# Jasonlai0821/fftw3

Measured on AMD Instinct MI355X. Metric: GFLOPS (5N*log2N) + achieved HBM GB/s, 1D complex double N=2^20 batch=4096, higher is better.
Workload: dtype f64; 1 GPU; c2c n=1048576 howmany=4096 per GPU, forward, out-of-place, FFTW_ESTIMATE; parallelism=batch-sharded x1

## Files before the change

fftw3_amd/csrc/fa_hip.h:

```cpp
#ifndef FA_HIP_H
#define FA_HIP_H

#include <stddef.h>
#include "fftw3_amd.h"

#ifdef __cplusplus
extern "C" {
#endif

int   fa_hip_device_count(void);
int   fa_hip_rr_tile(int L);
int   fa_hip_r3t_tile(int L);
int   fa_hip_r3tw_rdec(int L);
int   fa_hip_r2c_rows_tile(int L);
int   fa_hip_r2c_rows1_tile(int L);
int   fa_hip_r2c_rows2m_tile(int L);
int   fa_hip_r2c_rows3_tile(int L);
int   fa_hip_r3_tile(int L);
int   fa_hip_blue_nb(int need);
int   fa_hip_blue_tile(int nb);
int   fa_hip_r1_tile(int L);
void *fa_hip_malloc(size_t nbytes);
void  fa_hip_free(void *p);
void *fa_hip_host_malloc(size_t nbytes);
int   fa_hip_host_free(void *p);
int   fa_hip_is_device_ptr(const void *p);
int   fa_hip_ptr_device(const void *p);
void  fa_hip_memcpy_h2d(void *dst, const void *src, size_t nbytes, void *stream);
void  fa_hip_memcpy_d2h(void *dst, const void *src, size_t nbytes, void *stream);
void  fa_hip_memset(void *dst, int v, size_t nbytes, void *stream);
void  fa_hip_stream_sync(void *stream);
void *fa_hip_event_create(void);
void  fa_hip_event_record(void *ev, void *stream);
float fa_hip_event_elapsed_ms(void *start, void *stop);
void  fa_hip_event_destroy(void *ev);
void *fa_hip_stream_create(void);
void  fa_hip_stream_destroy(void *stream);
void  fa_hip_stream_wait_event(void *stream, void *ev);
int   fa_hip_get_device(void);
void  fa_hip_set_device(int dev);
int   fa_hip_enable_peer(int dev, int peer);
void  fa_hip_memcpy_peer(void *dst, int dst_dev, const void *src, int src_dev, size_t nbytes, void *stream);
void  fa_hip_memcpy2d_peer(void *dst, size_t dpitch, const void *src, size_t spitch, size_t width, size_t height, void *stream);
size_t fa_hip_max_pitch(int dev);

int   fa_hip_slab_twiddle(double *p, long long rows, long long width, long long row_stride, long long c0,
                          long long n, int sign, const void *lo, const void *hi, int shift, void *stream);

int fa_hip_launch_step(const fftw_amd_step_desc *desc, double *const *bufs,
                       void *const *tables, long long chunk_start, long long chunk_n,
                       void *stream);

int fa_hip_launch_pair1024(const fftw_amd_step_desc *d_second, double *const *bufs_second,
                           long long cs2, long long cn2,
                           const fftw_amd_step_desc *d_first, double *const *bufs_first,
                           long long cs1, long long cn1, void *const *tables, void *stream);

// ... 5 lines not shown
```

fftw3_amd/csrc/fa_plan.h:

```cpp
#ifndef FA_PLAN_H
#define FA_PLAN_H

#include <stddef.h>
#include <pthread.h>
#include "fftw3.h"
#include "fftw3_amd.h"

typedef long long i64;

#define FA_MAXRANK 8
#define FA_MAXLOOPS 7
#define FA_MAXBUF 16
#define FA_MAXTAB 256
#define FA_MAXPASS 4
#define FA_MAXLANES 4

#define FA_PRIME_LDS_MAX 31

#define FA_TILE_ELEMS 4096
#define FA_LMAX_SINGLE 4096
#define FA_LDS_ELEMS 5120

enum { FA_C2C = 0, FA_R2C = 1, FA_C2R = 2, FA_R2R = 3 };
#define FA_REAL_IN(t)  ((t) == FA_R2C || (t) == FA_R2R)
#define FA_REAL_OUT(t) ((t) == FA_C2R || (t) == FA_R2R)

enum {
    FA_TAB_STAGE = 1,
    FA_TAB_TW_LO,
    FA_TAB_TW_HI,
    FA_TAB_CHIRP,
    FA_TAB_BLUE_SEQ,
    FA_TAB_RADER_SEQ,
    FA_TAB_DFT_OF,
    FA_TAB_PERM
};

typedef struct {
    int kind;
    i64 n;
    i64 aux;
    i64 len;
    int src;
    void *host;
    void *dev;
} fa_table;

typedef struct { i64 n, is, os; } fa_dim;

typedef struct {
    size_t chunk_bytes;
    int pipeline;
    int lmax_multi;
    int small_tiles;
    int long_first;
    int lanes;
    i64 tile_elems;
    int real_dec;
} fa_cfg;

typedef struct {
    int buf;
    i64 base;
    i64 im;
} fa_loc;

typedef struct {
    i64 n;
    i64 is, os;
    fa_loc src, dst;
    int nloops;
    fa_dim loops[FA_MAXLOOPS];
    int batch_loop;
    int flags_in, flags_out;
    int dense;
} fa_axis;

struct fftw_plan_s {
    int type;
    int kinds[FA_MAXRANK];
    fa_cfg cfg;
    int sign;
    unsigned flags;
    int rank;
    fa_dim dims[FA_MAXRANK];
    int hrank;
    fa_dim hdims[FA_MAXRANK];
    i64 in_im, out_im;

    fftw_amd_step_desc *steps;
    int nsteps, cap_steps;

    fa_table tabs[FA_MAXTAB];
    int ntabs;

    int nbufs;
    i64 buf_reals[FA_MAXBUF];
    int buf_busy[FA_MAXBUF];
    double *dbuf[FA_MAXBUF];

    i64 batch, chunk;

    double *ri, *ii, *ro, *io;
    i64 in_lo, in_hi, out_lo, out_hi;
    i64 out_written;
    int inplace;
    int single_chunk;
    int via_scratch;

    void *stream;
    int dev_ready;
    pthread_mutex_t lock;

    int nslots, split;
    int pair;
    int lanes;
    void *pstream[FA_MAXLANES];
    void *ev_a[4], *ev_b[4], *ev_begin, *ev_end[FA_MAXLANES];
    int failed;

    void *hstream[2];
    double *stage_in, *stage_out;
    size_t stage_in_bytes, stage_out_bytes;

    double est_flops;

    struct fftw_plan_s *alt;

    double *prof_ms;
    long long *prof_launches;
};

void fa_cexp(i64 m, i64 n, double out[2]);
i64  fa_mulmod(i64 x, i64 y, i64 p);
i64  fa_power_mod(i64 b, i64 e, i64 p);
int  fa_prime_factors(i64 n, i64 *primes, int *mult);
int  fa_is_prime(i64 n);
i64  fa_largest_prime_factor(i64 n);
i64  fa_find_generator(i64 p);
int  fa_lds_able(i64 n);
i64  fa_next_smooth(i64 n);
int  fa_radices(i64 L, int *rad);
int  fa_factor_passes(i64 n, int max_passes, i64 lmax_single, i64 lmax_multi, i64 *lens);
int  fa_factor_passes_pref(i64 n, int max_passes, i64 lmax_single, i64 lmax_multi, i64 *lens,
                           int (*tuned)(i64));

struct fftw_plan_s *fa_plan_new(void);
void fa_plan_free(struct fftw_plan_s *p);
int  fa_build(struct fftw_plan_s *p);
int  fa_device_init(struct fftw_plan_s *p);
void fa_run(struct fftw_plan_s *p, double *ri, double *ii, double *ro, double *io);
char *fa_sprint(const struct fftw_plan_s *p);
fa_cfg fa_default_cfg(void);

struct fftw_plan_s *fa_unaligned_twin(const struct fftw_plan_s *p);

#define FA_SLAB_MAXDEV 32
struct fa_slab1d;
void fa_slab1d_execute(struct fa_slab1d *d);
void fa_slab1d_sync(struct fa_slab1d *d);
void fa_slab1d_destroy(struct fa_slab1d *d);
fftw_plan fa_slab1d_local_plan(const struct fa_slab1d *d, int g, int which);
struct fftw_amd_slab_plan_s *fa_slab_wrap1d(struct fa_slab1d *d, int ndev);

#endif
```

fftw3_amd/csrc/hostmath.c:

```c
#include <math.h>
#include <stdlib.h>
#include <string.h>
#include "fa_plan.h"

void fa_cexp(i64 m, i64 n, double out[2]) {
    const double two_pi = 6.2831853071795864769252867665590057683943388;
    i64 full = 4 * n;
    i64 q = n;
    i64 a;
    int flip_s = 0, rot = 0, swap = 0;
    m %= n;
    if (m < 0) m += n;
    a = 4 * m;
    if (a > full - a) { a = full - a; flip_s = 1; }
    if (a > q) { a -= q; rot = 1; }
    if (a > q - a) { a = q - a; swap = 1; }
    {
        double th = (two_pi * (double)a) / (double)full;
        double c = cos(th), s = sin(th), t;
        if (swap) { t = c; c = s; s = t; }
        if (rot) { t = c; c = -s; s = t; }
        if (flip_s) s = -s;
        out[0] = c;
        out[1] = s;
    }
}

i64 fa_mulmod(i64 x, i64 y, i64 p) {
    return (i64)(((unsigned __int128)x * (unsigned __int128)y) % (unsigned __int128)p);
}

i64 fa_power_mod(i64 b, i64 e, i64 p) {
    i64 r = 1 % p;
    b %= p;
    if (b < 0) b += p;
    while (e > 0) {
        if (e & 1) r = fa_mulmod(r, b, p);
        b = fa_mulmod(b, b, p);
        e >>= 1;
    }
    return r;
}

int fa_prime_factors(i64 n, i64 *primes, int *mult) {
    int k = 0;
    i64 d;
    for (d = 2; d * d <= n; d += (d == 2 ? 1 : 2)) {
        if (n % d == 0) {
            primes[k] = d;
            mult[k] = 0;
            while (n % d == 0) { n /= d; ++mult[k]; }
            ++k;
        }
    }
    if (n > 1) { primes[k] = n; mult[k] = 1; ++k; }
    return k;
}

int fa_is_prime(i64 n) {
    i64 d;
    if (n < 2) return 0;
    for (d = 2; d * d <= n; d += (d == 2 ? 1 : 2))
        if (n % d == 0) return 0;
    return 1;
}

i64 fa_largest_prime_factor(i64 n) {
    i64 pr[64];
    int mu[64];
    int k = fa_prime_factors(n, pr, mu);
    return k ? pr[k - 1] : 1;
}

i64 fa_find_generator(i64 p) {
    i64 pr[64];
    int mu[64];
    int k, i;
    i64 g;
    if (p == 2) return 1;
    k = fa_prime_factors(p - 1, pr, mu);
// ... 174 lines not shown
```

fftw3_amd/csrc/kernels.hip:

```cpp
#include <string.h>
#include "common.hpp"

#include "pass1024.hpp"


struct PassArgs {
    const double *src;
    double *dst;
    i64 src_im, dst_im;
    i64 is_l, os_l;
    i64 dn[FFTW_AMD_MAX_DIMS], dis[FFTW_AMD_MAX_DIMS], dos[FFTW_AMD_MAX_DIMS], dtw[FFTW_AMD_MAX_DIMS];
    const cplx *wL;
    const cplx *tw_lo;
    const cplx *tw_hi;
    i64 tw_n;
    i64 ntiles;
    int tw_shift;
    int L, nrad;
    int rad[FFTW_AMD_MAX_RADICES];
    int ndims, T, ld, flags;
    int in_t_fast, out_t_fast;
    int lo_n;
    i64 lo_is, lo_os;
};
// ... 991 lines not shown
    if (e != hipSuccess) (void)hipGetLastError();
    FA_CHECK(hipSetDevice(cur));
    return (e == hipSuccess || e == hipErrorPeerAccessAlreadyEnabled) ? 0 : 1;
}
extern "C" void fa_hip_memcpy_peer(void *dst, int dst_dev, const void *src, int src_dev, size_t n, void *stream) {
    if (dst_dev == src_dev) FA_CHECK(hipMemcpyAsync(dst, src, n, hipMemcpyDeviceToDevice, (hipStream_t)stream));
    else FA_CHECK(hipMemcpyPeerAsync(dst, dst_dev, src, src_dev, n, (hipStream_t)stream));
}
extern "C" void fa_hip_memcpy2d_peer(void *dst, size_t dpitch, const void *src, size_t spitch, size_t width, size_t height, void *stream) {
    if (!width || !height) return;
    FA_CHECK(hipMemcpy2DAsync(dst, dpitch, src, spitch, width, height, hipMemcpyDeviceToDevice, (hipStream_t)stream));
}
extern "C" void fa_hip_stream_wait_event(void *s, void *ev) {
    FA_CHECK(hipStreamWaitEvent((hipStream_t)s, (hipEvent_t)ev, 0));
}


static void grid_for(i64 total, dim3 *grid) {
    i64 blocks = (total + 255) / 256;
    if (blocks < 1) blocks = 1;
    if (blocks > 256 * 32) blocks = 256 * 32;
    *grid = dim3((unsigned)blocks, 1, 1);
}


static std::atomic<unsigned> g_lds_attr_done{0};

template <bool VIN, bool VOUT>
static void launch_pass_variant(const PassArgs &pa, dim3 grid, size_t lds, hipStream_t st) {
    static int nth = 0;
    if (!nth) { const char *e = getenv("FFTW_AMD_GENERIC_THREADS"); nth = e ? atoi(e) : 256; if (nth < 64 || nth > 256) nth = 256; }
    hipLaunchKernelGGL((pass_generic_kernel<VIN, VOUT>), grid, dim3(nth), lds, st, pa);
}

int fa_launch_pass3tw(const fftw_amd_step_desc *d, double *const *bufs, void *const *tables,
                      i64 cs, i64 cn, hipStream_t st);
int fa_launch_pass3gw(const fftw_amd_step_desc *d, double *const *bufs, void *const *tables,
                      i64 cs, i64 cn, hipStream_t st);
int fa_launch_pass3g(const fftw_amd_step_desc *d, double *const *bufs, void *const *tables,
                     i64 cs, i64 cn, hipStream_t st);
int fa_launch_pass3t(const fftw_amd_step_desc *d, double *const *bufs, void *const *tables,
                     i64 cs, i64 cn, hipStream_t st);
int fa_launch_r2crows(const fftw_amd_step_desc *d, double *const *bufs, void *const *tables,
                      i64 cs, i64 cn, hipStream_t st);
int fa_launch_pass3s(const fftw_amd_step_desc *d, double *const *bufs, void *const *tables,
                     i64 cs, i64 cn, hipStream_t st);
int fa_launch_passrr(const fftw_amd_step_desc *d, double *const *bufs, void *const *tables,
                     i64 cs, i64 cn, hipStream_t st);
int fa_launch_blue(const fftw_amd_step_desc *d, double *const *bufs, void *const *tables,
                   i64 cs, i64 cn, hipStream_t st);
int fa_launch_pass1r(const fftw_amd_step_desc *d, double *const *bufs, void *const *tables,
                     i64 cs, i64 cn, hipStream_t st);

template <bool IN_T, bool OUT_T, int HAS_TW>
static void launch_p1024_variant(const P1024Args &pa, dim3 grid, hipStream_t st) {
    static std::atomic<unsigned> attr_done{0};
    const size_t lds = FA_P1024_LDS_DOUBLES * sizeof(double);
    if (fa_attr_needed(attr_done)) {
        FA_CHECK(hipFuncSetAttribute((const void *)pass1024_kernel<IN_T, OUT_T, HAS_TW>,
                                     hipFuncAttributeMaxDynamicSharedMemorySize, (int)lds));
        fa_attr_set(attr_done);
    }
    hipLaunchKernelGGL((pass1024_kernel<IN_T, OUT_T, HAS_TW>), grid, dim3(256), lds, st, pa);
}

static int fill_p1024(const fftw_amd_step_desc *d, double *const *bufs, void *const *tables,
                      i64 cs, i64 cn, P1024Args &pa, i64 *nblocks_out, bool *in_t, bool *out_t, int *tw) {
    int bd = d->batch_dim;
    i64 sbase = d->src_base, dbase = d->dst_base;
    if (d->L != 1024 || d->src_im != 1 || d->dst_im != 1 ||
        (d->flags & (FFTW_AMD_F_REAL_IN | FFTW_AMD_F_REAL_OUT | FFTW_AMD_F_CONJ_OUT)))
        return 1;
    for (int i = 0; i < FFTW_AMD_MAX_DIMS; ++i) {
        pa.dn[i] = (i < d->ndims) ? d->dim_n[i] : 1;
        pa.dis[i] = (i < d->ndims) ? d->dim_is[i] : 0;
        pa.dos[i] = (i < d->ndims) ? d->dim_os[i] : 0;
        pa.dtw[i] = (i < d->ndims) ? d->dim_tw[i] : 0;
    }
    if (bd >= 0) {
        sbase += chunk_adv(d->src_buf, cs, d->dim_is[bd]);
        dbase += chunk_adv(d->dst_buf, cs, d->dim_os[bd]);
        pa.dn[bd] = cn;
    }
    pa.src = bufs[d->src_buf] + sbase;
    pa.dst = bufs[d->dst_buf] + dbase;
    pa.is_l = d->is_l;
    pa.os_l = d->os_l;
    if (((uintptr_t)pa.src % 16) || ((uintptr_t)pa.dst % 16) || (pa.is_l % 2) || (pa.os_l % 2)) return 1;
    for (int i = 0; i < d->ndims; ++i)
        if ((pa.dis[i] % 2) || (pa.dos[i] % 2)) return 1;
    pa.w1024 = (const cplx *)tables[d->table];
    pa.tw_shift = d->tw_shift;
    pa.tw_lo = d->tw_n ? (const cplx *)tables[d->tw_lo] : NULL;
    pa.tw_hi = d->tw_n ? (const cplx *)tables[d->tw_hi] : NULL;
    pa.ndims = d->ndims;
    pa.flags = d->flags;
    pa.lo_sh = 0; pa.lo_is = d->tile_lo_is; pa.lo_os = d->tile_lo_os;
    pa.dbg = NULL;
    if (d->tile_lo_n > 1) {
        if (d->tile_lo_n != 2 && d->tile_lo_n != 4) return 1;
        pa.lo_sh = d->tile_lo_n == 2 ? 1 : 2;
        if ((pa.lo_is % 2) || (pa.lo_os % 2)) return 1;
    }
    pa.ntiles = (pa.dn[0] + (8 >> pa.lo_sh) - 1) / (8 >> pa.lo_sh);
    i64 nblocks = pa.ntiles;
    for (int i = 1; i < d->ndims; ++i) nblocks *= pa.dn[i];
    if (nblocks > 0x7fffffffLL) return 1;
    *nblocks_out = nblocks < 0 ? 0 : nblocks;
    *in_t = pa.dn[0] > 1 && iabs64(pa.dis[0]) <= iabs64(pa.is_l);
    *out_t = pa.dn[0] > 1 && iabs64(pa.dos[0]) <= iabs64(pa.os_l);
    *tw = d->tw_n == 0 ? 0 : ((d->flags & FFTW_AMD_F_TW_IN) ? 2 : 1);
    return 0;
}

static int launch_p1024(const fftw_amd_step_desc *d, double *const *bufs, void *const *tables,
                        i64 cs, i64 cn, hipStream_t st) {
    P1024Args pa;
    i64 nblocks = 0;
    bool in_t, out_t;
    int tw;
    if (fill_p1024(d, bufs, tables, cs, cn, pa, &nblocks, &in_t, &out_t, &tw)) return 1;
    if (nblocks <= 0) return 0;
    dim3 grid((unsigned)nblocks, 1, 1);
#define FA_P1024_CASE(I, O, W) if (in_t == I && out_t == O && tw == W) { launch_p1024_variant<I, O, W>(pa, grid, st); return 0; }
    FA_P1024_CASE(true, true, 0)  FA_P1024_CASE(true, true, 1)  FA_P1024_CASE(true, true, 2)
    FA_P1024_CASE(false, true, 0) FA_P1024_CASE(false, true, 1) FA_P1024_CASE(false, true, 2)
    FA_P1024_CASE(true, false, 0) FA_P1024_CASE(true, false, 1) FA_P1024_CASE(true, false, 2)
    FA_P1024_CASE(false, false, 0) FA_P1024_CASE(false, false, 1) FA_P1024_CASE(false, false, 2)
#undef FA_P1024_CASE
    return 1;
}

template <bool IN_T, bool OUT_T, int HAS_TW>
FA_DEV void p1024_block(const P1024Args &a, unsigned b0, unsigned nb, double *plane) {
    unsigned blk = (nb & 7) ? b0 : (b0 & 7) * (nb >> 3) + (b0 >> 3);
    const unsigned nt = (unsigned)a.ntiles;
    unsigned rest = blk / nt;
    const unsigned tile = blk - rest * nt;
    i64 soff = 0, doff = 0, twb = 0;
    for (int d = 1; d < a.ndims; ++d) {
        const unsigned dn = (unsigned)a.dn[d];
        const unsigned q = rest / dn, idx = rest - q * dn;
        rest = q;
        soff += (i64)idx * a.dis[d];
        doff += (i64)idx * a.dos[d];
        twb += (i64)idx * a.dtw[d];
    }
    const i64 t0 = (i64)tile * 8;
    P1024Tile t;
    t.lo_sh = 0; t.lo_is = 0; t.lo_os = 0;
    t.src = a.src + soff + t0 * a.dis[0];
    t.dst = a.dst + doff + t0 * a.dos[0];
    t.is_l = a.is_l; t.os_l = a.os_l;
    t.dis0 = a.dis[0]; t.dos0 = a.dos[0];
    t.dtw0 = a.dtw[0]; t.q0 = twb + t0 * a.dtw[0];
    t.w1024 = a.w1024; t.tw_lo = a.tw_lo; t.tw_hi = a.tw_hi; t.tw_shift = a.tw_shift;
    t.Tcur = (int)((a.dn[0] - t0 < 8) ? (a.dn[0] - t0) : 8);
    t.flags = a.flags;
    t.dbg = NULL;
    p1024_tile<IN_T, OUT_T, HAS_TW, 0>(t, plane, threadIdx.x);
}

__global__ void __launch_bounds__(256, 2)
pass1024_pair_kernel(const P1024Args a2, const P1024Args a1, const unsigned n2, const unsigned n1) {
    extern __shared__ __attribute__((aligned(16))) double plane[];
    if (blockIdx.x < n2) p1024_block<false, true, 2>(a2, blockIdx.x, n2, plane);
    else p1024_block<true, true, 0>(a1, blockIdx.x - n2, n1, plane);
}

extern "C" int fa_hip_launch_pair1024(const fftw_amd_step_desc *d_second, double *const *bufs_second,
                                      long long cs2, long long cn2,
                                      const fftw_amd_step_desc *d_first, double *const *bufs_first,
                                      long long cs1, long long cn1, void *const *tables, void *stream) {
    P1024Args a2, a1;
    i64 n2 = 0, n1 = 0;
    bool i2 = false, o2 = true, i1 = true, o1 = true;
    int w2 = 2, w1 = 0;
    memset((void *)&a2, 0, sizeof(a2));
    memset((void *)&a1, 0, sizeof(a1));
    if (cn2 > 0 && fill_p1024(d_second, bufs_second, tables, cs2, cn2, a2, &n2, &i2, &o2, &w2)) return 1;
    if (cn1 > 0 && fill_p1024(d_first, bufs_first, tables, cs1, cn1, a1, &n1, &i1, &o1, &w1)) return 1;
    if ((cn2 > 0 && (i2 || !o2 || w2 != 2 || a2.lo_sh)) || (cn1 > 0 && (!i1 || !o1 || w1 != 0 || a1.lo_sh))) return 1;
    if (n1 + n2 <= 0) return 0;
    if (n1 + n2 > 0x7fffffffLL) return 1;
    static std::atomic<unsigned> attr_done{0};
    const size_t lds = FA_P1024_LDS_DOUBLES * sizeof(double);
    if (fa_attr_needed(attr_done)) {
        FA_CHECK(hipFuncSetAttribute((const void *)pass1024_pair_kernel, hipFuncAttributeMaxDynamicSharedMemorySize, (int)lds));
        fa_attr_set(attr_done);
    }
    hipLaunchKernelGGL(pass1024_pair_kernel, dim3((unsigned)(n1 + n2)), dim3(256), lds, (hipStream_t)stream,
                       a2, a1, (unsigned)n2, (unsigned)n1);
    hipError_t e = hipGetLastError();
    if (e != hipSuccess) { fprintf(stderr, "fftw3_amd: pair launch failed: %s\n", hipGetErrorString(e)); return -1; }
    return 0;
}

static int launch_pass(const fftw_amd_step_desc *d, double *const *bufs, void *const *tables,
                       i64 cs, i64 cn, hipStream_t st) {
    PassArgs pa;
    if (d->flags & (FFTW_AMD_F_R2C_ROWS | FFTW_AMD_F_C2R_ROWS)) return fa_launch_r2crows(d, bufs, tables, cs, cn, st);
    if (d->flags & FFTW_AMD_F_REAL_DEC) {
        if (fa_launch_pass3tw(d, bufs, tables, cs, cn, st) == 0) return 0;
        fprintf(stderr, "fftw3_amd: internal error: real-decimated rows step with an unsupported layout\n");
        abort();
    }
    if (d->variant == FFTW_AMD_K_P1024 && launch_p1024(d, bufs, tables, cs, cn, st) == 0) return 0;
    if (d->variant == FFTW_AMD_K_BLUE) return fa_launch_blue(d, bufs, tables, cs, cn, st);
    if (d->variant == FFTW_AMD_K_R1 && fa_launch_pass1r(d, bufs, tables, cs, cn, st) == 0) return 0;
    if (d->variant == FFTW_AMD_K_RR && fa_launch_passrr(d, bufs, tables, cs, cn, st) == 0) return 0;
    if (d->variant == FFTW_AMD_K_R3 && d->L > 8192 && d->L < 16384 && fa_launch_pass3gw(d, bufs, tables, cs, cn, st) == 0) return 0;
    if (d->variant == FFTW_AMD_K_R3 && d->L > 1024 && d->L <= 2048 && fa_launch_pass3tw(d, bufs, tables, cs, cn, st) == 0) return 0;
    if (d->variant == FFTW_AMD_K_R3 && (fa_launch_pass3s(d, bufs, tables, cs, cn, st) == 0 ||
                                        fa_launch_pass3g(d, bufs, tables, cs, cn, st) == 0 ||
                                        fa_launch_pass3t(d, bufs, tables, cs, cn, st) == 0)) return 0;
    int bd = d->batch_dim;
    i64 sbase = d->src_base, dbase = d->dst_base;
    for (int i = 0; i < FFTW_AMD_MAX_DIMS; ++i) {
        pa.dn[i] = (i < d->ndims) ? d->dim_n[i] : 1;
        pa.dis[i] = (i < d->ndims) ? d->dim_is[i] : 0;
        pa.dos[i] = (i < d->ndims) ? d->dim_os[i] : 0;
        pa.dtw[i] = (i < d->ndims) ? d->dim_tw[i] : 0;
    }
    if (bd >= 0) {
        sbase += chunk_adv(d->src_buf, cs, d->dim_is[bd]);
        dbase += chunk_adv(d->dst_buf, cs, d->dim_os[bd]);
        pa.dn[bd] = cn;
    }
    pa.src = bufs[d->src_buf] + sbase;
    pa.dst = bufs[d->dst_buf] + dbase;
    pa.src_im = d->src_im;
    pa.dst_im = d->dst_im;
    pa.is_l = d->is_l;
    pa.os_l = d->os_l;
    pa.wL = (d->table >= 0) ? (const cplx *)tables[d->table] : NULL;
    pa.tw_n = d->tw_n;
    pa.tw_shift = d->tw_shift;
    pa.tw_lo = d->tw_n ? (const cplx *)tables[d->tw_lo] : NULL;
    pa.tw_hi = d->tw_n ? (const cplx *)tables[d->tw_hi] : NULL;
    pa.L = d->L;
    pa.nrad = d->nradices;
    for (int i = 0; i < FFTW_AMD_MAX_RADICES; ++i) pa.rad[i] = (i < d->nradices) ? d->radices[i] : 1;
    pa.ndims = d->ndims;
    pa.T = d->tile;
    pa.lo_n = d->tile_lo_n > 1 ? d->tile_lo_n : 1;
// ... 414 lines not shown
```

fftw3_amd/csrc/pass1024.hpp:

```cpp
#ifndef FA_PASS1024_HPP
#define FA_PASS1024_HPP

template <int M> struct W32 {
    static constexpr double cs[32] = {
        1.0, 0.98078528040323044912618223613423903697393373089333, 0.92387953251128675612818318939678828682241662586364,
        0.83146961230254523707878837761790575673856081198797, 0.70710678118654752440084436210484903928483593768847,
        0.55557023301960222474283081394853287437493719075480, 0.38268343236508977172845998403039886676134456248563,
        0.19509032201612826784828486847702224092769161775195, 0.0, -0.19509032201612826784828486847702224092769161775195,
        -0.38268343236508977172845998403039886676134456248563, -0.55557023301960222474283081394853287437493719075480,
        -0.70710678118654752440084436210484903928483593768847, -0.83146961230254523707878837761790575673856081198797,
        -0.92387953251128675612818318939678828682241662586364, -0.98078528040323044912618223613423903697393373089333,
        -1.0, -0.98078528040323044912618223613423903697393373089333, -0.92387953251128675612818318939678828682241662586364,
        -0.83146961230254523707878837761790575673856081198797, -0.70710678118654752440084436210484903928483593768847,
        -0.55557023301960222474283081394853287437493719075480, -0.38268343236508977172845998403039886676134456248563,
        -0.19509032201612826784828486847702224092769161775195, 0.0, 0.19509032201612826784828486847702224092769161775195,
        0.38268343236508977172845998403039886676134456248563, 0.55557023301960222474283081394853287437493719075480,
        0.70710678118654752440084436210484903928483593768847, 0.83146961230254523707878837761790575673856081198797,
        0.92387953251128675612818318939678828682241662586364, 0.98078528040323044912618223613423903697393373089333
    };
    static constexpr double c = cs[M & 31];
    static constexpr double s = cs[(M + 24) & 31];
};

template <int M> FA_DEV cplx mul_w32c(cplx v) {
// ... 22 lines not shown
        x[I + 12] = mul_w32c<I * 3>(e[3]);
        x[I + 16] = mul_w32c<I * 4>(e[4]);
        x[I + 20] = mul_w32c<I * 5>(e[5]);
        x[I + 24] = mul_w32c<I * 6>(e[6]);
        x[I + 28] = mul_w32c<I * 7>(e[7]);
    }
};

FA_DEV void bfly32(cplx *x) {
    Bfly32Step1<0>::run(x);
    Bfly32Step1<1>::run(x);
    Bfly32Step1<2>::run(x);
    Bfly32Step1<3>::run(x);
#pragma unroll
    for (int k2 = 0; k2 < 8; ++k2) {
        cplx c[4] = { x[4 * k2], x[4 * k2 + 1], x[4 * k2 + 2], x[4 * k2 + 3] };
        Bfly<4>::run(c);
        x[4 * k2] = c[0]; x[4 * k2 + 1] = c[1]; x[4 * k2 + 2] = c[2]; x[4 * k2 + 3] = c[3];
    }
}

template <int BIT, int D, bool HAVE, bool PERM> struct TwTree {
    static FA_DEV void run(cplx *x, const cplx *pw, cplx acc) {
        TwTree<BIT - 1, D, HAVE, PERM>::run(x, pw, acc);
        cplx nxt = HAVE ? c_mul(acc, pw[BIT]) : pw[BIT];
        TwTree<BIT - 1, D + (1 << BIT), true, PERM>::run(x, pw, nxt);
    }
};
template <int D, bool HAVE, bool PERM> struct TwTree<-1, D, HAVE, PERM> {
    static FA_DEV void run(cplx *x, const cplx *, cplx acc) {
        constexpr int S = PERM ? slot32(D) : D;
        if (HAVE) x[S] = c_mulc(x[S], acc);
    }
};

template <bool IN_T, bool OUT_T> FA_DEV int lds_index(int d, int a, int t) {
    if (IN_T && OUT_T) return d * 264 + a * 8 + t;
    if (!IN_T && OUT_T) return d * 264 + t * 33 + a;
    if (IN_T && !OUT_T) return a * 264 + t * 33 + d;
    return t * 1056 + d * 33 + a;
}

#define FA_P1024_LDS_DOUBLES 8448

struct P1024Tile {
    const double *src;
    double *dst;
    i64 is_l, os_l;
    i64 dis0, dos0;
    i64 dtw0, q0;
    const cplx *w1024;
    const cplx *tw_lo;
    const cplx *tw_hi;
    int tw_shift;
    int Tcur;
    int flags;
    int lo_sh;
    i64 lo_is, lo_os;
    long long *dbg;
};

#define FA_TILE_SOFF(a, t) ((i64)((t) >> (a).lo_sh) * (a).dis0 + (i64)((t) & ((1 << (a).lo_sh) - 1)) * (a).lo_is)
#define FA_TILE_DOFF(a, t) ((i64)((t) >> (a).lo_sh) * (a).dos0 + (i64)((t) & ((1 << (a).lo_sh) - 1)) * (a).lo_os)

template <bool IN_T, bool OUT_T, int HAS_TW, int ABL = 0>
FA_DEV void p1024_tile(const P1024Tile &a, double *plane, const int tid) {
    const int ti = IN_T ? (tid & 7) : (tid >> 5);
    const int ai = IN_T ? (tid >> 3) : (tid & 31);
    const int to = OUT_T ? (tid & 7) : (tid >> 5);
    const int dq = OUT_T ? (tid >> 3) : (tid & 31);

    cplx pw1024[5];
#pragma unroll
    for (int s = 0; s < 5; ++s) pw1024[s] = (ABL & 2) ? c_make(1.0, 0.0) : a.w1024[ai << s];
    cplx twl[6], twh[6];
    if (HAS_TW != 0 && !(ABL & 2)) {
        const i64 q = a.q0 + (i64)((HAS_TW == 2 ? ti : to) >> a.lo_sh) * a.dtw0;
        const i64 mask = (1LL << a.tw_shift) - 1;
        const i64 m0 = q * (HAS_TW == 2 ? ai : dq);
        twl[5] = a.tw_lo[m0 & mask]; twh[5] = a.tw_hi[m0 >> a.tw_shift];
#pragma unroll
        for (int s = 0; s < 5; ++s) {
            const i64 m = (q * 32) << s;
            twl[s] = a.tw_lo[m & mask]; twh[s] = a.tw_hi[m >> a.tw_shift];
        }
    }
    cplx x[32];
    {
        const double *p = a.src + (i64)ai * a.is_l + FA_TILE_SOFF(a, ti);
        const i64 step = 32 * a.is_l;
        if ((ti >> a.lo_sh) >= a.Tcur) {
#pragma unroll
            for (int i = 0; i < 32; ++i) x[i] = c_make(0.0, 0.0);
        } else if (a.flags & FFTW_AMD_F_NT_IN) {
#pragma unroll
            for (int i = 0; i < 32; ++i) x[i] = ld_cplx<true>(p + i * step);
        } else {
#pragma unroll
            for (int i = 0; i < 32; ++i) x[i] = ld_cplx<false>(p + i * step);
        }
        if (a.flags & FFTW_AMD_F_SWAP_IN) {
#pragma unroll
            for (int i = 0; i < 32; ++i) { double s = x[i].x; x[i].x = x[i].y; x[i].y = s; }
        }
    }
    if (ABL & 8) {
        asm volatile("s_waitcnt vmcnt(0)" ::: "memory");
        if (tid == 0) a.dbg[1] = wall_clock64();
    }

    if (HAS_TW == 2 && !(ABL & 2)) {
        cplx base = c_mul(twl[5], twh[5]);
        cplx pw[5];
#pragma unroll
        for (int s = 0; s < 5; ++s) pw[s] = c_mul(twl[s], twh[s]);
        TwTree<4, 0, true, false>::run(x, pw, base);
    }

    if (!(ABL & 1)) bfly32(x);
    if (!(ABL & 2)) TwTree<4, 0, false, true>::run(x, pw1024, c_make(1.0, 0.0));

    cplx y[32];
    if (ABL & 4) {
#pragma unroll
        for (int q = 0; q < 32; ++q) y[q] = x[slot32(q)];
    } else {
#pragma unroll
    for (int d = 0; d < 32; ++d) plane[lds_index<IN_T, OUT_T>(d, ai, ti)] = x[slot32(d)].x;
    __syncthreads();
#pragma unroll
    for (int q = 0; q < 32; ++q) y[q].x = plane[lds_index<IN_T, OUT_T>(dq, q, to)];
    __syncthreads();
#pragma unroll
    for (int d = 0; d < 32; ++d) plane[lds_index<IN_T, OUT_T>(d, ai, ti)] = x[slot32(d)].y;
    __syncthreads();
#pragma unroll
    for (int q = 0; q < 32; ++q) y[q].y = plane[lds_index<IN_T, OUT_T>(dq, q, to)];
    }

    if (!(ABL & 1)) bfly32(y);

    if (HAS_TW == 1 && !(ABL & 2)) {
        cplx base = c_mul(twl[5], twh[5]);
        cplx pw[5];
#pragma unroll
        for (int s = 0; s < 5; ++s) pw[s] = c_mul(twl[s], twh[s]);
        TwTree<4, 0, true, true>::run(y, pw, base);
    }

    if ((ABL & 8) && tid == 0) a.dbg[2] = wall_clock64();
    if ((to >> a.lo_sh) < a.Tcur) {
        double *p = a.dst + (i64)dq * a.os_l + FA_TILE_DOFF(a, to);
        const i64 step = 32 * a.os_l;
        const bool sw = (a.flags & FFTW_AMD_F_SWAP_OUT) != 0;
        if (a.flags & FFTW_AMD_F_NT_OUT) {
#pragma unroll
            for (int c = 0; c < 32; ++c) {
                cplx v = y[slot32(c)];
                if (sw) { double s = v.x; v.x = v.y; v.y = s; }
                st_cplx<true>(p + c * step, v);
            }
        } else {
#pragma unroll
            for (int c = 0; c < 32; ++c) {
                cplx v = y[slot32(c)];
                if (sw) { double s = v.x; v.x = v.y; v.y = s; }
                st_cplx<false>(p + c * step, v);
            }
        }
    }
    if (ABL & 8) {
        if (tid == 0) a.dbg[3] = wall_clock64();
        asm volatile("s_waitcnt vmcnt(0)" ::: "memory");
        if (tid == 0) a.dbg[4] = wall_clock64();
        if ((tid & 63) == 0) a.dbg[12 + (tid >> 6)] = wall_clock64();
    }
}

struct P1024Args {
    const double *src;
    double *dst;
    i64 is_l, os_l;
    i64 dn[FFTW_AMD_MAX_DIMS], dis[FFTW_AMD_MAX_DIMS], dos[FFTW_AMD_MAX_DIMS], dtw[FFTW_AMD_MAX_DIMS];
    const cplx *w1024;
    const cplx *tw_lo;
    const cplx *tw_hi;
    i64 ntiles;
    int tw_shift;
    int ndims, flags;
    int lo_sh;
    i64 lo_is, lo_os;
    long long *dbg;
};

template <bool IN_T, bool OUT_T, int HAS_TW, int ABL = 0>
__global__ void __launch_bounds__(256, 2)
pass1024_kernel(const P1024Args a) {
    extern __shared__ __attribute__((aligned(16))) double plane[];
    long long t_first = 0;
    if (ABL & 8) t_first = wall_clock64();
    unsigned blk = (unsigned)fa_xcd_remap((i64)blockIdx.x, (i64)gridDim.x);
    const unsigned nt = (unsigned)a.ntiles;
    unsigned tile = blk % nt;
    unsigned rest = blk / nt;
    i64 soff = 0, doff = 0, twb = 0;
    for (int d = 1; d < a.ndims; ++d) {
        const unsigned dn = (unsigned)a.dn[d];
        unsigned idx = rest % dn;
        rest /= dn;
        soff += (i64)idx * a.dis[d];
        doff += (i64)idx * a.dos[d];
        twb += (i64)idx * a.dtw[d];
    }
    const i64 t0 = (i64)tile * (8 >> a.lo_sh);
    P1024Tile t;
    t.lo_sh = a.lo_sh; t.lo_is = a.lo_is; t.lo_os = a.lo_os;
    t.src = a.src + soff + t0 * a.dis[0];
    t.dst = a.dst + doff + t0 * a.dos[0];
    t.is_l = a.is_l; t.os_l = a.os_l;
    t.dis0 = a.dis[0]; t.dos0 = a.dos[0];
    t.dtw0 = a.dtw[0]; t.q0 = twb + t0 * a.dtw[0];
    t.w1024 = a.w1024; t.tw_lo = a.tw_lo; t.tw_hi = a.tw_hi; t.tw_shift = a.tw_shift;
    t.Tcur = (int)((a.dn[0] - t0 < (8 >> a.lo_sh)) ? (a.dn[0] - t0) : (8 >> a.lo_sh));
    t.flags = a.flags;
    t.dbg = NULL;
    if (ABL & 8) {
        t.dbg = a.dbg + (i64)blockIdx.x * 16;
        if (threadIdx.x == 0) {
            unsigned hw;
            asm volatile("s_getreg_b32 %0, hwreg(HW_REG_HW_ID)" : "=s"(hw));
            unsigned xcc;
            asm volatile("s_getreg_b32 %0, hwreg(HW_REG_XCC_ID)" : "=s"(xcc));
            t.dbg[0] = wall_clock64();
            t.dbg[5] = hw; t.dbg[6] = xcc; t.dbg[7] = (long long)blk; t.dbg[8] = t_first;
        }
    }
    p1024_tile<IN_T, OUT_T, HAS_TW, ABL>(t, plane, threadIdx.x);
}

#endif
```

fftw3_amd/csrc/planner.c:

```c
#include <math.h>
#include <stdarg.h>
#include <stdio.h>
#include <stdlib.h>
#include <string.h>
#include "fa_plan.h"
#include "fa_hip.h"

typedef struct fftw_plan_s plan;

#define FA_DEFAULT_CHUNK_BYTES ((size_t)128 << 20)
static size_t g_chunk_bytes = FA_DEFAULT_CHUNK_BYTES;

void fftw_amd_set_chunk_bytes(size_t nbytes) {
    __atomic_store_n(&g_chunk_bytes, nbytes ? nbytes : FA_DEFAULT_CHUNK_BYTES, __ATOMIC_RELAXED);
}

static i64 iabs(i64 v) { return v < 0 ? -v : v; }

fa_cfg fa_default_cfg(void) {
    fa_cfg c;
    const char *e;
    c.chunk_bytes = __atomic_load_n(&g_chunk_bytes, __ATOMIC_RELAXED);
    c.pipeline = 0;
    c.lmax_multi = 1024;
    c.small_tiles = 1;
    c.long_first = 0;
    c.tile_elems = 0;
    c.real_dec = 0;
    c.lanes = 2;
    e = getenv("FFTW_AMD_CHUNK_BYTES");
    if (e && atoll(e) > 0) c.chunk_bytes = (size_t)atoll(e);
    e = getenv("FFTW_AMD_SMALL_TILES");
    if (e) c.small_tiles = atoi(e);
    e = getenv("FFTW_AMD_TILE_ELEMS");
    if (e) c.tile_elems = atoll(e);
    e = getenv("FFTW_AMD_LONG_FIRST");
    if (e) c.long_first = atoi(e);
    e = getenv("FFTW_AMD_PIPELINE");
    if (e) c.pipeline = atoi(e);
    e = getenv("FFTW_AMD_LMAX_MULTI");
    if (e && atoll(e) >= 16) c.lmax_multi = (int)atoll(e);
    e = getenv("FFTW_AMD_REAL_DEC");
    if (e) c.real_dec = atoi(e) != 0;
    e = getenv("FFTW_AMD_LANES");
    if (e && atoi(e) >= 1 && atoi(e) <= FA_MAXLANES) c.lanes = atoi(e);
    return c;
}


plan *fa_plan_new(void) {
    plan *p = (plan *)calloc(1, sizeof(plan));
    if (!p) return NULL;
    p->nbufs = 2;
    p->in_im = p->out_im = 1;
    p->cfg = fa_default_cfg();
    pthread_mutex_init(&p->lock, NULL);
    return p;
}

static void plan_reset_build(plan *p) {
    int i;
    free(p->steps);
    p->steps = NULL;
    p->nsteps = p->cap_steps = 0;
    for (i = 0; i < p->ntabs; ++i) free(p->tabs[i].host);
    memset(p->tabs, 0, sizeof(p->tabs));
    p->ntabs = 0;
    p->nbufs = 2;
    memset(p->buf_reals, 0, sizeof(p->buf_reals));
    memset(p->buf_busy, 0, sizeof(p->buf_busy));
    p->failed = 0;
    p->est_flops = 0;
}

void fa_plan_free(plan *p) {
    int i;
    if (!p) return;
    if (p->alt) { fa_plan_free(p->alt); p->alt = NULL; }
    {
        int any = p->dev_ready || p->stage_in || p->stage_out || p->hstream[0] || p->pstream[0];
        for (i = 0; i < p->ntabs && !any; ++i) any = p->tabs[i].dev != NULL;
        for (i = 2; i < p->nbufs && !any; ++i) any = p->dbuf[i] != NULL;
        if (!any) goto host_only;
    }
    {
        fa_hip_stream_sync(p->stream);
        for (i = 0; i < p->ntabs; ++i) fa_hip_free(p->tabs[i].dev);
        for (i = 2; i < p->nbufs; ++i) fa_hip_free(p->dbuf[i]);
        fa_hip_free(p->stage_in);
        fa_hip_free(p->stage_out);
        if (p->hstream[0]) fa_hip_stream_destroy(p->hstream[0]);
        if (p->hstream[1]) fa_hip_stream_destroy(p->hstream[1]);
        if (p->pstream[0]) {
            for (i = 0; i < 4; ++i) { if (p->ev_a[i]) fa_hip_event_destroy(p->ev_a[i]); if (p->ev_b[i]) fa_hip_event_destroy(p->ev_b[i]); }
            fa_hip_event_destroy(p->ev_begin);
            for (i = 0; i < FA_MAXLANES; ++i) {
                if (p->ev_end[i]) fa_hip_event_destroy(p->ev_end[i]);
                if (p->pstream[i]) fa_hip_stream_destroy(p->pstream[i]);
// ... 12 lines not shown
    int i;
    for (i = 0; i < p->ntabs; ++i)
        if (p->tabs[i].kind == kind && p->tabs[i].n == n && p->tabs[i].aux == aux) return i;
    return -1;
}

static int tab_new(plan *p, int kind, i64 n, i64 aux, i64 len, size_t elem) {
    fa_table *t;
    if (p->ntabs >= FA_MAXTAB) { p->failed = 1; return 0; }
    t = &p->tabs[p->ntabs];
    t->kind = kind;
    t->n = n;
    t->aux = aux;
    t->len = len;
    t->src = -1;
    t->host = len ? calloc((size_t)len, elem) : NULL;
    t->dev = NULL;
    return p->ntabs++;
}

static int tab_stage(plan *p, i64 L) {
    int id = tab_find(p, FA_TAB_STAGE, L, 0);
    double *h;
    i64 m;
    if (id >= 0) return id;
    id = tab_new(p, FA_TAB_STAGE, L, 0, L, 2 * sizeof(double));
    h = (double *)p->tabs[id].host;
    for (m = 0; m < L; ++m) fa_cexp(m, L, h + 2 * m);
    return id;
}

static void tab_tw2(plan *p, i64 n, int *lo, int *hi, int *shift) {
    int s = 0, id;
    i64 m, nlo, nhi;
    double *h;
    while (((i64)1 << (2 * s)) < n) ++s;
    nlo = (i64)1 << s;
    nhi = (n + nlo - 1) / nlo;
    *shift = s;
    id = tab_find(p, FA_TAB_TW_LO, n, s);
    if (id < 0) {
        id = tab_new(p, FA_TAB_TW_LO, n, s, nlo, 2 * sizeof(double));
        h = (double *)p->tabs[id].host;
        for (m = 0; m < nlo; ++m) fa_cexp(m, n, h + 2 * m);
    }
    *lo = id;
    id = tab_find(p, FA_TAB_TW_HI, n, s);
    if (id < 0) {
        id = tab_new(p, FA_TAB_TW_HI, n, s, nhi, 2 * sizeof(double));
        h = (double *)p->tabs[id].host;
        for (m = 0; m < nhi; ++m) fa_cexp(m << s, n, h + 2 * m);
    }
    *hi = id;
}

static int tab_chirp(plan *p, i64 n, i64 nb) {
    int id = tab_find(p, FA_TAB_CHIRP, n, nb);
    double *h;
    i64 k;
    if (id >= 0) return id;
    id = tab_new(p, FA_TAB_CHIRP, n, nb, nb, 2 * sizeof(double));
    h = (double *)p->tabs[id].host;
    for (k = 0; k < n; ++k) fa_cexp(fa_mulmod(k, k, 2 * n), 2 * n, h + 2 * k);
    return id;
}

static int tab_dft_of(plan *p, int src, i64 n) {
    int id = tab_find(p, FA_TAB_DFT_OF, n, src);
    if (id >= 0) return id;
    id = tab_new(p, FA_TAB_DFT_OF, n, src, n, 2 * sizeof(double));
    free(p->tabs[id].host);
    p->tabs[id].host = NULL;
    p->tabs[id].src = src;
    return id;
}

static int tab_blue_kernel(plan *p, i64 n, i64 nb) {
    int seq = tab_find(p, FA_TAB_BLUE_SEQ, n, nb);
    if (seq < 0) {
        double *h, w[2];
        i64 k;
        seq = tab_new(p, FA_TAB_BLUE_SEQ, n, nb, nb, 2 * sizeof(double));
        h = (double *)p->tabs[seq].host;
        for (k = 0; k < n; ++k) {
            fa_cexp(fa_mulmod(k, k, 2 * n), 2 * n, w);
            h[2 * k] = w[0] / (double)nb;
            h[2 * k + 1] = w[1] / (double)nb;
            if (k) {
                h[2 * (nb - k)] = h[2 * k];
                h[2 * (nb - k) + 1] = h[2 * k + 1];
            }
        }
    }
    return tab_dft_of(p, seq, nb);
}

static int tab_perm(plan *p, i64 pr, int inverse) {
    int id = tab_find(p, FA_TAB_PERM, pr, inverse);
    i64 *h, g, x, k;
    if (id >= 0) return id;
    id = tab_new(p, FA_TAB_PERM, pr, inverse, pr - 1, sizeof(i64));
    h = (i64 *)p->tabs[id].host;
    g = fa_find_generator(pr);
    if (inverse) g = fa_power_mod(g, pr - 2, pr);
    x = 1;
    for (k = 0; k < pr - 1; ++k) {
// ... 153 lines not shown
    s->L = (int)L;
    s->is_l = is_l;
    s->os_l = os_l;
    s->nradices = fa_radices(L, s->radices);
    if (s->nradices < 0) { p->failed = 1; return; }
    if (L > 1) s->table = tab_stage(p, L);
    if (best < 0) {
        sdim tmp[FFTW_AMD_MAX_DIMS + 1];
        memset(&dummy, 0, sizeof(dummy));
        dummy.n = 1;
        tmp[0] = dummy;
        for (i = 0; i < nd && i < FFTW_AMD_MAX_DIMS; ++i) tmp[i + 1] = dims[i];
        step_set_dims(p, s, tmp, nd + 1, 0);
    } else {
        step_set_dims(p, s, dims, nd, best);
    }
    T = FA_TILE_ELEMS / L;
    {
        i64 elems = p->cfg.tile_elems > 0 ? p->cfg.tile_elems : (p->cfg.small_tiles ? 1024 : FA_TILE_ELEMS);
        i64 cap = elems / L, floor_t = (iabs(is_l) <= 2 && iabs(os_l) <= 2) ? 1 : 8;
        if (cap < floor_t) cap = floor_t;
        if (T > cap) T = cap;
    }
    if (T < 1) T = 1;
    if (T > s->dim_n[0] * s->tile_lo_n) T = s->dim_n[0] * s->tile_lo_n;
    while (T > 1 && L * (T | 1) > FA_LDS_ELEMS) --T;
    T -= T % s->tile_lo_n;
    if (T < 1) T = 1;
    s->tile = (int)T;
    if (src.im == 1 && dst.im == 1 && !(flags & (FFTW_AMD_F_REAL_IN | FFTW_AMD_F_REAL_OUT)) &&
        !getenv("FFTW_AMD_NO_TUNED")) {
        if (L == 1024) {
            s->variant = FFTW_AMD_K_P1024;
            s->tile = 8;
        } else if (L <= 32 && fa_hip_r1_tile((int)L) > 0 && is_l == 2 && os_l == 2 && tw_n == 0 && s->tile_lo_n == 1 &&
                   s->dim_is[0] == 2 * L && s->dim_os[0] == 2 * L && s->dim_n[0] >= 256 && !getenv("FFTW_AMD_NO_R1")) {
            s->variant = FFTW_AMD_K_R1;
            s->tile = fa_hip_r1_tile((int)L);
        } else if (fa_hip_r3_tile((int)L) > 0 && is_l == 2 && os_l == 2 && tw_n == 0 && s->tile_lo_n == 1 &&
                   (L == 2048 || L == 4096 || L == 8192 || L == 16384 || s->dim_n[0] * 2 >= fa_hip_r3_tile((int)L))) {
            s->variant = FFTW_AMD_K_R3;
            s->tile = fa_hip_r3_tile((int)L);
        } else if (fa_hip_rr_tile((int)L) > 0 && s->dim_n[0] * s->tile_lo_n * 4 >= fa_hip_rr_tile((int)L) &&
                   (s->tile_lo_n == 1 || (L & (L - 1)) == 0)) {
            s->variant = FFTW_AMD_K_RR;
            s->tile = fa_hip_rr_tile((int)L);
        } else if (fa_hip_r3t_tile((int)L) > 0 && s->tile_lo_n == 1 && s->dim_n[0] * 4 >= fa_hip_r3t_tile((int)L)) {
            s->variant = FFTW_AMD_K_R3;
            s->tile = fa_hip_r3t_tile((int)L);
        }
    }
    s->tw_n = tw_n;
    if (tw_n) tab_tw2(p, tw_n, &s->tw_lo, &s->tw_hi, &s->tw_shift);
    {
        double work = (double)L;
        for (i = 0; i < s->ndims; ++i) work *= (double)s->dim_n[i];
        if (L > 1) p->est_flops += 5.0 * work * log2((double)L);
        if (tw_n) p->est_flops += 6.0 * work;
    }
}

static void emit_copy(plan *p, int kind, fa_loc src, fa_loc dst, i64 K, i64 Kvalid,
                      i64 is_k, i64 os_k, const sdim *dims, int nd, int flags,
                      int table, int table2) {
    fftw_amd_step_desc *s = new_step(p, kind);
    s->src_buf = src.buf; s->src_base = src.base; s->src_im = src.im;
    s->dst_buf = dst.buf; s->dst_base = dst.base; s->dst_im = dst.im;
    s->flags = flags;
    s->is_l = is_k;
    s->os_l = os_k;
    s->aux_n = K;
    s->aux_valid = Kvalid;
    s->table = table;
    s->table2 = table2;
    step_set_dims(p, s, dims, nd, -1);
}


static void fa_emit_axis(plan *p, const fa_axis *ax);
static int has_register_kernel(i64 L);

static int loops_to_sdims(const fa_axis *ax, sdim *d, int use_dst_as_src) {
    int i;
    for (i = 0; i < ax->nloops; ++i) {
        d[i].n = ax->loops[i].n;
        d[i].is = use_dst_as_src ? ax->loops[i].os : ax->loops[i].is;
        d[i].os = ax->loops[i].os;
        d[i].tw = 0;
        d[i].is_batch = (i == ax->batch_loop);
    }
    return ax->nloops;
}

static i64 scratch_layout_u(const fa_axis *ax, i64 n_axis, i64 unit, i64 *ts_axis, i64 *ts_loop) {
    int order[FA_MAXLOOPS + 1], cnt = 0, i, j;
    i64 key[FA_MAXLOOPS + 1], stride = unit;
    order[cnt] = -1;
    key[cnt] = iabs(ax->is);
    ++cnt;
    for (i = 0; i < ax->nloops; ++i) {
        if (i == ax->batch_loop) continue;
        order[cnt] = i;
        key[cnt] = iabs(ax->loops[i].is);
        ++cnt;
    }
    for (i = 1; i < cnt; ++i) {
// ... 2014 lines not shown
```

Before: 9944 GFLOPS.

## Precompute per-sequence twiddle table for pass1024 input-twiddle kernel

Adds a host-built per-sequence twiddle table holding 32 per-lane twiddles and 5 power-of-two step twiddles for each sequence index, computed in long double. The pass1024 kernel with input twiddles reads these directly instead of combining lo/hi split tables with complex multiplies and power chains. This reduces twiddle arithmetic and scattered table gathers at the cost of an extra table (capped at 1024 sequences) and new template variants. An env var keeps the old path available.

```diff
diff --git a/fftw3_amd/csrc/fa_hip.h b/fftw3_amd/csrc/fa_hip.h
--- a/fftw3_amd/csrc/fa_hip.h
+++ b/fftw3_amd/csrc/fa_hip.h
@@ -3,6 +3,8 @@
 
 #include <stddef.h>
 #include "fftw3_amd.h"
+
+#define FA_P1024_TWQ_STRIDE 40
 
 #ifdef __cplusplus
 extern "C" {
diff --git a/fftw3_amd/csrc/fa_plan.h b/fftw3_amd/csrc/fa_plan.h
--- a/fftw3_amd/csrc/fa_plan.h
+++ b/fftw3_amd/csrc/fa_plan.h
@@ -33,7 +33,8 @@
     FA_TAB_BLUE_SEQ,
     FA_TAB_RADER_SEQ,
     FA_TAB_DFT_OF,
-    FA_TAB_PERM
+    FA_TAB_PERM,
+    FA_TAB_TWQ
 };
 
 typedef struct {
@@ -56,6 +57,7 @@
     int long_first;
     int lanes;
     i64 tile_elems;
+    int p1024_v1;
     int real_dec;
 } fa_cfg;
 
@@ -132,6 +134,7 @@
 };
 
 void fa_cexp(i64 m, i64 n, double out[2]);
+void fa_cexp_ld(i64 m, i64 n, double out[2]);
 i64  fa_mulmod(i64 x, i64 y, i64 p);
 i64  fa_power_mod(i64 b, i64 e, i64 p);
 int  fa_prime_factors(i64 n, i64 *primes, int *mult);
diff --git a/fftw3_amd/csrc/hostmath.c b/fftw3_amd/csrc/hostmath.c
--- a/fftw3_amd/csrc/hostmath.c
+++ b/fftw3_amd/csrc/hostmath.c
@@ -26,6 +26,27 @@
     }
 }
 
+void fa_cexp_ld(i64 m, i64 n, double out[2]) {
+    const long double two_pi = 6.2831853071795864769252867665590057683943388L;
+    i64 full = 4 * n, q = n, a;
+    int flip_s = 0, rot = 0, swap = 0;
+    m %= n;
+    if (m < 0) m += n;
+    a = 4 * m;
+    if (a > full - a) { a = full - a; flip_s = 1; }
+    if (a > q) { a -= q; rot = 1; }
+    if (a > q - a) { a = q - a; swap = 1; }
+    {
+        long double th = (two_pi * (long double)a) / (long double)full;
+        long double c = cosl(th), s = sinl(th), t;
+        if (swap) { t = c; c = s; s = t; }
+        if (rot) { t = c; c = -s; s = t; }
+        if (flip_s) s = -s;
+        out[0] = (double)c;
+        out[1] = (double)s;
+    }
+}
+
 i64 fa_mulmod(i64 x, i64 y, i64 p) {
     return (i64)(((unsigned __int128)x * (unsigned __int128)y) % (unsigned __int128)p);
 }
diff --git a/fftw3_amd/csrc/kernels.hip b/fftw3_amd/csrc/kernels.hip
--- a/fftw3_amd/csrc/kernels.hip
+++ b/fftw3_amd/csrc/kernels.hip
@@ -1067,16 +1067,26 @@
 int fa_launch_pass1r(const fftw_amd_step_desc *d, double *const *bufs, void *const *tables,
                      i64 cs, i64 cn, hipStream_t st);
 
-template <bool IN_T, bool OUT_T, int HAS_TW>
-static void launch_p1024_variant(const P1024Args &pa, dim3 grid, hipStream_t st) {
+template <bool IN_T, bool OUT_T, int HAS_TW, bool TWQ>
+static void launch_p1024_body(const P1024Args &pa, dim3 grid, hipStream_t st) {
     static std::atomic<unsigned> attr_done{0};
     const size_t lds = FA_P1024_LDS_DOUBLES * sizeof(double);
     if (fa_attr_needed(attr_done)) {
-        FA_CHECK(hipFuncSetAttribute((const void *)pass1024_kernel<IN_T, OUT_T, HAS_TW>,
+        FA_CHECK(hipFuncSetAttribute((const void *)pass1024_kernel<IN_T, OUT_T, HAS_TW, 0, TWQ>,
                                      hipFuncAttributeMaxDynamicSharedMemorySize, (int)lds));
         fa_attr_set(attr_done);
     }
-    hipLaunchKernelGGL((pass1024_kernel<IN_T, OUT_T, HAS_TW>), grid, dim3(256), lds, st, pa);
+    hipLaunchKernelGGL((pass1024_kernel<IN_T, OUT_T, HAS_TW, 0, TWQ>), grid, dim3(256), lds, st, pa);
+}
+
+template <bool IN_T, bool OUT_T, int HAS_TW>
+static void launch_p1024_variant(const P1024Args &pa, dim3 grid, hipStream_t st) {
+    if constexpr (HAS_TW == 2) {
+        if (pa.twq != NULL) launch_p1024_body<IN_T, OUT_T, HAS_TW, true>(pa, grid, st);
+        else launch_p1024_body<IN_T, OUT_T, HAS_TW, false>(pa, grid, st);
+    } else {
+        launch_p1024_body<IN_T, OUT_T, HAS_TW, false>(pa, grid, st);
+    }
 }
 
 static int fill_p1024(const fftw_amd_step_desc *d, double *const *bufs, void *const *tables,
@@ -1108,6 +1118,7 @@
     pa.tw_shift = d->tw_shift;
     pa.tw_lo = d->tw_n ? (const cplx *)tables[d->tw_lo] : NULL;
     pa.tw_hi = d->tw_n ? (const cplx *)tables[d->tw_hi] : NULL;
+    pa.twq = (d->tw_n && (d->flags & FFTW_AMD_F_TW_IN) && d->table2 >= 0) ? (const cplx *)tables[d->table2] : NULL;
     pa.ndims = d->ndims;
     pa.flags = d->flags;
     pa.lo_sh = 0; pa.lo_is = d->tile_lo_is; pa.lo_os = d->tile_lo_os;
@@ -1146,7 +1157,7 @@
     return 1;
 }
 
-template <bool IN_T, bool OUT_T, int HAS_TW>
+template <bool IN_T, bool OUT_T, int HAS_TW, bool TWQ>
 FA_DEV void p1024_block(const P1024Args &a, unsigned b0, unsigned nb, double *plane) {
     unsigned blk = (nb & 7) ? b0 : (b0 & 7) * (nb >> 3) + (b0 >> 3);
     const unsigned nt = (unsigned)a.ntiles;
@@ -1169,18 +1180,31 @@
     t.is_l = a.is_l; t.os_l = a.os_l;
     t.dis0 = a.dis[0]; t.dos0 = a.dos[0];
     t.dtw0 = a.dtw[0]; t.q0 = twb + t0 * a.dtw[0];
-    t.w1024 = a.w1024; t.tw_lo = a.tw_lo; t.tw_hi = a.tw_hi; t.tw_shift = a.tw_shift;
+    t.w1024 = a.w1024; t.tw_lo = a.tw_lo; t.tw_hi = a.tw_hi; t.twq = a.twq; t.tw_shift = a.tw_shift;
     t.Tcur = (int)((a.dn[0] - t0 < 8) ? (a.dn[0] - t0) : 8);
     t.flags = a.flags;
     t.dbg = NULL;
-    p1024_tile<IN_T, OUT_T, HAS_TW, 0>(t, plane, threadIdx.x);
-}
-
+    p1024_tile<IN_T, OUT_T, HAS_TW, 0, TWQ>(t, plane, threadIdx.x);
+}
+
+template <bool TWQ>
 __global__ void __launch_bounds__(256, 2)
 pass1024_pair_kernel(const P1024Args a2, const P1024Args a1, const unsigned n2, const unsigned n1) {
     extern __shared__ __attribute__((aligned(16))) double plane[];
-    if (blockIdx.x < n2) p1024_block<false, true, 2>(a2, blockIdx.x, n2, plane);
-    else p1024_block<true, true, 0>(a1, blockIdx.x - n2, n1, plane);
+    if (blockIdx.x < n2) p1024_block<false, true, 2, TWQ>(a2, blockIdx.x, n2, plane);
+    else p1024_block<true, true, 0, false>(a1, blockIdx.x - n2, n1, plane);
+}
+
+template <bool TWQ>
+static void launch_pair1024_body(const P1024Args &a2, const P1024Args &a1, unsigned n2, unsigned n1, hipStream_t st) {
+    static std::atomic<unsigned> attr_done{0};
+    const size_t lds = FA_P1024_LDS_DOUBLES * sizeof(double);
+    if (fa_attr_needed(attr_done)) {
+        FA_CHECK(hipFuncSetAttribute((const void *)pass1024_pair_kernel<TWQ>, hipFuncAttributeMaxDynamicSharedMemorySize,
+                                     (int)lds));
+        fa_attr_set(attr_done);
+    }
+    hipLaunchKernelGGL((pass1024_pair_kernel<TWQ>), dim3(n1 + n2), dim3(256), lds, st, a2, a1, n2, n1);
 }
 
 extern "C" int fa_hip_launch_pair1024(const fftw_amd_step_desc *d_second, double *const *bufs_second,
@@ -1198,14 +1222,8 @@
     if ((cn2 > 0 && (i2 || !o2 || w2 != 2 || a2.lo_sh)) || (cn1 > 0 && (!i1 || !o1 || w1 != 0 || a1.lo_sh))) return 1;
     if (n1 + n2 <= 0) return 0;
     if (n1 + n2 > 0x7fffffffLL) return 1;
-    static std::atomic<unsigned> attr_done{0};
-    const size_t lds = FA_P1024_LDS_DOUBLES * sizeof(double);
-    if (fa_attr_needed(attr_done)) {
-        FA_CHECK(hipFuncSetAttribute((const void *)pass1024_pair_kernel, hipFuncAttributeMaxDynamicSharedMemorySize, (int)lds));
-        fa_attr_set(attr_done);
-    }
-    hipLaunchKernelGGL(pass1024_pair_kernel, dim3((unsigned)(n1 + n2)), dim3(256), lds, (hipStream_t)stream,
-                       a2, a1, (unsigned)n2, (unsigned)n1);
+    if (cn2 > 0 && a2.twq != NULL) launch_pair1024_body<true>(a2, a1, (unsigned)n2, (unsigned)n1, (hipStream_t)stream);
+    else launch_pair1024_body<false>(a2, a1, (unsigned)n2, (unsigned)n1, (hipStream_t)stream);
     hipError_t e = hipGetLastError();
     if (e != hipSuccess) { fprintf(stderr, "fftw3_amd: pair launch failed: %s\n", hipGetErrorString(e)); return -1; }
     return 0;
diff --git a/fftw3_amd/csrc/pass1024.hpp b/fftw3_amd/csrc/pass1024.hpp
--- a/fftw3_amd/csrc/pass1024.hpp
+++ b/fftw3_amd/csrc/pass1024.hpp
@@ -98,6 +98,7 @@
     const cplx *w1024;
     const cplx *tw_lo;
     const cplx *tw_hi;
+    const cplx *twq;
     int tw_shift;
     int Tcur;
     int flags;
@@ -109,7 +110,7 @@
 #define FA_TILE_SOFF(a, t) ((i64)((t) >> (a).lo_sh) * (a).dis0 + (i64)((t) & ((1 << (a).lo_sh) - 1)) * (a).lo_is)
 #define FA_TILE_DOFF(a, t) ((i64)((t) >> (a).lo_sh) * (a).dos0 + (i64)((t) & ((1 << (a).lo_sh) - 1)) * (a).lo_os)
 
-template <bool IN_T, bool OUT_T, int HAS_TW, int ABL = 0>
+template <bool IN_T, bool OUT_T, int HAS_TW, int ABL = 0, bool TWQ = false>
 FA_DEV void p1024_tile(const P1024Tile &a, double *plane, const int tid) {
     const int ti = IN_T ? (tid & 7) : (tid >> 5);
     const int ai = IN_T ? (tid >> 3) : (tid & 31);
@@ -119,8 +120,15 @@
     cplx pw1024[5];
 #pragma unroll
     for (int s = 0; s < 5; ++s) pw1024[s] = (ABL & 2) ? c_make(1.0, 0.0) : a.w1024[ai << s];
+    static_assert(!TWQ || HAS_TW == 2, "the per-sequence table serves the input twiddle");
     cplx twl[6], twh[6];
-    if (HAS_TW != 0 && !(ABL & 2)) {
+    if (TWQ && !(ABL & 2)) {
+        const i64 q = ((ti >> a.lo_sh) < a.Tcur) ? a.q0 + (i64)(ti >> a.lo_sh) * a.dtw0 : 0;
+        const cplx *r = a.twq + q * FA_P1024_TWQ_STRIDE;
+        twl[5] = r[ai];
+#pragma unroll
+        for (int s = 0; s < 5; ++s) twl[s] = r[32 + s];
+    } else if (HAS_TW != 0 && !(ABL & 2)) {
         const i64 q = a.q0 + (i64)((HAS_TW == 2 ? ti : to) >> a.lo_sh) * a.dtw0;
         const i64 mask = (1LL << a.tw_shift) - 1;
         const i64 m0 = q * (HAS_TW == 2 ? ai : dq);
@@ -155,7 +163,9 @@
         if (tid == 0) a.dbg[1] = wall_clock64();
     }
 
-    if (HAS_TW == 2 && !(ABL & 2)) {
+    if (TWQ && !(ABL & 2)) {
+        TwTree<4, 0, true, false>::run(x, twl, twl[5]);
+    } else if (HAS_TW == 2 && !(ABL & 2)) {
         cplx base = c_mul(twl[5], twh[5]);
         cplx pw[5];
 #pragma unroll
@@ -231,6 +241,7 @@
     const cplx *w1024;
     const cplx *tw_lo;
     const cplx *tw_hi;
+    const cplx *twq;
     i64 ntiles;
     int tw_shift;
     int ndims, flags;
@@ -239,7 +250,7 @@
     long long *dbg;
 };
 
-template <bool IN_T, bool OUT_T, int HAS_TW, int ABL = 0>
+template <bool IN_T, bool OUT_T, int HAS_TW, int ABL = 0, bool TWQ = false>
 __global__ void __launch_bounds__(256, 2)
 pass1024_kernel(const P1024Args a) {
     extern __shared__ __attribute__((aligned(16))) double plane[];
@@ -266,7 +277,7 @@
     t.is_l = a.is_l; t.os_l = a.os_l;
     t.dis0 = a.dis[0]; t.dos0 = a.dos[0];
     t.dtw0 = a.dtw[0]; t.q0 = twb + t0 * a.dtw[0];
-    t.w1024 = a.w1024; t.tw_lo = a.tw_lo; t.tw_hi = a.tw_hi; t.tw_shift = a.tw_shift;
+    t.w1024 = a.w1024; t.tw_lo = a.tw_lo; t.tw_hi = a.tw_hi; t.twq = a.twq; t.tw_shift = a.tw_shift;
     t.Tcur = (int)((a.dn[0] - t0 < (8 >> a.lo_sh)) ? (a.dn[0] - t0) : (8 >> a.lo_sh));
     t.flags = a.flags;
     t.dbg = NULL;
@@ -281,7 +292,7 @@
             t.dbg[5] = hw; t.dbg[6] = xcc; t.dbg[7] = (long long)blk; t.dbg[8] = t_first;
         }
     }
-    p1024_tile<IN_T, OUT_T, HAS_TW, ABL>(t, plane, threadIdx.x);
+    p1024_tile<IN_T, OUT_T, HAS_TW, ABL, TWQ>(t, plane, threadIdx.x);
 }
 
 #endif
diff --git a/fftw3_amd/csrc/planner.c b/fftw3_amd/csrc/planner.c
--- a/fftw3_amd/csrc/planner.c
+++ b/fftw3_amd/csrc/planner.c
@@ -44,6 +44,8 @@
     if (e) c.real_dec = atoi(e) != 0;
     e = getenv("FFTW_AMD_LANES");
     if (e && atoi(e) >= 1 && atoi(e) <= FA_MAXLANES) c.lanes = atoi(e);
+    e = getenv("FFTW_AMD_P1024_V1");
+    c.p1024_v1 = e && atoi(e) != 0;
     return c;
 }
 
@@ -162,6 +164,29 @@
         for (m = 0; m < nhi; ++m) fa_cexp(m << s, n, h + 2 * m);
     }
     *hi = id;
+}
+
+#define FA_TWQ_MAX_Q 1024
+static int tab_twq(plan *p, const fftw_amd_step_desc *s, i64 n) {
+    i64 Q = 1, q;
+    int i, id, a, k;
+    double *h;
+    for (i = 0; i < s->ndims; ++i) {
+        if (s->dim_tw[i] < 0 || s->dim_n[i] < 1) return -1;
+        Q += (s->dim_n[i] - 1) * s->dim_tw[i];
+        if (Q > FA_TWQ_MAX_Q) return -1;
+    }
+    id = tab_find(p, FA_TAB_TWQ, n, Q);
+    if (id >= 0) return id;
+    id = tab_new(p, FA_TAB_TWQ, n, Q, FA_P1024_TWQ_STRIDE * Q, 2 * sizeof(double));
+    h = (double *)p->tabs[id].host;
+    if (!h) return -1;
+    for (q = 0; q < Q; ++q) {
+        double *r = h + 2 * FA_P1024_TWQ_STRIDE * q;
+        for (a = 0; a < 32; ++a) fa_cexp_ld(q * a, n, r + 2 * a);
+        for (k = 0; k < 5; ++k) fa_cexp_ld((32 * q) << k, n, r + 2 * (32 + k));
+    }
+    return id;
 }
 
 static int tab_chirp(plan *p, i64 n, i64 nb) {
@@ -421,6 +446,8 @@
     }
     s->tw_n = tw_n;
     if (tw_n) tab_tw2(p, tw_n, &s->tw_lo, &s->tw_hi, &s->tw_shift);
+    if (s->variant == FFTW_AMD_K_P1024 && tw_n && (flags & FFTW_AMD_F_TW_IN) && !p->cfg.p1024_v1)
+        s->table2 = tab_twq(p, s, tw_n);
     {
         double work = (double)L;
         for (i = 0; i < s->ndims; ++i) work *= (double)s->dim_n[i];
```

After: 10090 GFLOPS, median of 6. 1.4% higher.
